# pxl-th/SLAM.jl

Measured on AMD Instinct MI355X. Metric: frames/sec KITTI-05 stereo @1k kpts; local-BA ms/iter for 50-KF window, higher is better.
Workload: dtype f64

## Files before the change

slam.jl_amd/csrc/detect.hip:

```cpp
#include "kpset.hpp"
#include "geom_device.hpp"
#include <cmath>
#include <cstddef>

#define DET_THREADS 256
#define DET_MAXCAND 512
#define DET_MAXTAPS 41
#define DET_MAXR 64

struct DetectArgs {
    const double *img; int H, W, pitch;
    const double *cur; int n_cur;
    int radius, grid_rows, grid_cols, cs, k;
    double min_response;
    int ntaps;
    double taps[DET_MAXTAPS];
    int64_t *cell_out;
    int *cell_cnt;
    const int *cur_off, *k_s; size_t zs; int kmax;
    const int *cur_cnt; int cur_stride, max_points;
    signed char lim[DET_MAXR + 1];
};
static void det_disk_table(DetectArgs &A)
{
    const int r = A.radius;
    for (int dy = 0; dy <= DET_MAXR; dy++) A.lim[dy] = -1;
    for (int dy = 0; dy <= r && dy <= DET_MAXR; dy++) {
        const volatile double a = (double)dy / (double)r;
        int lim = -1;
        for (int dx = 0; dx <= r; dx++) {
            const volatile double b = (double)dx / (double)r;
            const volatile double aa = a * a, bb = b * b;
            if (aa + bb < 1) lim = dx; else break;
        }
        A.lim[dy] = (signed char)lim;
    }
}

__device__ __forceinline__ int clampi(int v, int lo, int hi) { return v < lo ? lo : (v > hi ? hi : v); }

__device__ __forceinline__ double sep3(const double *src, int h, int w, int y, int x,
                                       double ky0, double ky1, double ky2, double kx0, double kx1, double kx2)
{
    const int ym = clampi(y - 1, 0, h - 1), yp = clampi(y + 1, 0, h - 1);
    double t[3];
#pragma unroll
    for (int j = 0; j < 3; j++) {
        const int xx = clampi(x + j - 1, 0, w - 1);
        double acc = 0.0;
        acc += src[ym + xx * h] * ky0; acc += src[y + xx * h] * ky1; acc += src[yp + xx * h] * ky2;
        t[j] = acc;
    }
    double acc = 0.0;
    acc += t[0] * kx0; acc += t[1] * kx1; acc += t[2] * kx2;
    return acc;
}

#define DET_SL 5
struct DetDiv {
    unsigned m, d;
    __device__ __forceinline__ explicit DetDiv(int dd) : m(0xffffffffu / (unsigned)(dd > 0 ? dd : 1) + 1u), d((unsigned)(dd > 0 ? dd : 1)) {}
    __device__ __forceinline__ int div(int i) const { return d == 1 ? i : (int)__umulhi((unsigned)i, m); }
    __device__ __forceinline__ int mod(int i) const { return i - div(i) * (int)d; }
};
template <int NT>
__device__ __forceinline__ void blur_mask(double *bA, double *T, const unsigned char *m0, const double *taps, int h, int w, int mh, int mw, int tid, const DetDiv &dns, const DetDiv &dh, int ntaps = NT)
{
    const int nt = NT > 0 ? NT : ntaps;
    if (NT > 0) {
        constexpr int NK = NT > 0 ? NT : 1;
        double k[NK];
#pragma unroll
        for (int j = 0; j < NK; j++) k[j] = taps[j];
        const int ns = (h + DET_SL - 1) / DET_SL;
        for (int it = tid; it < mw * ns; it += DET_THREADS) {
            const int tx = dns.div(it), ys = (it - tx * ns) * DET_SL;
            double v[DET_SL + NK - 1];
#pragma unroll
            for (int i = 0; i < DET_SL + NK - 1; i++) { const int yy = ys + i < mh ? ys + i : mh - 1; v[i] = (double)m0[yy + tx * mh]; }
#pragma unroll
            for (int q = 0; q < DET_SL; q++) {
                if (ys + q < h) {
                    double acc = 0.0;
#pragma unroll
                    for (int j = 0; j < NK; j++) acc += v[q + j] * k[j];
                    T[(ys + q) + tx * h] = acc;
                }
            }
        }
        __syncthreads();
        const int nsx = (w + DET_SL - 1) / DET_SL;
        for (int it = tid; it < h * nsx; it += DET_THREADS) {
            const int sx = dh.div(it), y = it - sx * h, xs = sx * DET_SL;
            double v[DET_SL + NK - 1];
#pragma unroll
            for (int i = 0; i < DET_SL + NK - 1; i++) { const int xx = xs + i < mw ? xs + i : mw - 1; v[i] = T[y + xx * h]; }
#pragma unroll
            for (int q = 0; q < DET_SL; q++) {
                if (xs + q < w) {
                    double acc = 0.0;
#pragma unroll
                    for (int j = 0; j < NK; j++) acc += v[q + j] * k[j];
                    bA[y + (xs + q) * h] = bA[y + (xs + q) * h] * acc;
                }
            }
        }
        return;
    }
    for (int i = tid; i < h * mw; i += DET_THREADS) {
        const int tx = dh.div(i), y = i - tx * h;
        double acc = 0.0;
        for (int j = 0; j < nt; j++) acc += (double)m0[(y + j) + tx * mh] * taps[j];
        T[i] = acc;
    }
    __syncthreads();
    for (int i = tid; i < h * w; i += DET_THREADS) {
        const int x = dh.div(i), y = i - x * h;
        double acc = 0.0;
        for (int j = 0; j < nt; j++) acc += T[y + (x + j) * h] * taps[j];
        bA[i] = bA[i] * acc;
    }
}

struct DetStrip { double v[3][DET_SL + 2]; };
__device__ __forceinline__ void det_strip_load(DetStrip &S, const double *src, int h, int w, int ys, int x)
{
    const int xm = clampi(x - 1, 0, w - 1), xp = clampi(x + 1, 0, w - 1);
#pragma unroll
    for (int i = 0; i < DET_SL + 2; i++) {
        const int yy = clampi(ys - 1 + i, 0, h - 1);
        S.v[0][i] = src[yy + xm * h]; S.v[1][i] = src[yy + x * h]; S.v[2][i] = src[yy + xp * h];
    }
}
__device__ __forceinline__ double det_strip_sep3(const DetStrip &S, int q, double ky0, double ky1, double ky2, double kx0, double kx1, double kx2)
{
    double t[3];
#pragma unroll
    for (int j = 0; j < 3; j++) {
        double acc = 0.0;
        acc += S.v[j][q] * ky0; acc += S.v[j][q + 1] * ky1; acc += S.v[j][q + 2] * ky2;
        t[j] = acc;
    }
    double acc = 0.0;
    acc += t[0] * kx0; acc += t[1] * kx1; acc += t[2] * kx2;
    return acc;
}

#ifdef DET_TRACE
#define DT(k) do { __syncthreads(); dt_clk[k] = clock64() - dt_t0; } while (0)
#else
#define DT(k)
#endif
#define SEL_NAME(k) k
#define SEL_ARG
#define SEL_STREAM(b) b
#include "detect_kernels.inc"
#undef SEL_NAME
#undef SEL_ARG
#undef SEL_STREAM
#define SEL_NAME(k) k##_sel
#define SEL_ARG , const int *stream_sel
#define SEL_STREAM(b) stream_sel[b]
#include "detect_kernels.inc"
#undef SEL_NAME
#undef SEL_ARG
#undef SEL_STREAM

__global__ __launch_bounds__(1024) void detect_compact(const int64_t *cell_out, const int *cell_cnt, int n_cells, int k,
                                                        int64_t *out , int cap,
                                                        const int *k_s )
{
    if (k_s) {
        const int z = blockIdx.x;
        cell_out += (size_t)z * n_cells * k * 2; cell_cnt += (size_t)z * n_cells; out += (size_t)z * (1 + 2 * (size_t)cap);
        k = k_s[z];
    }
    __shared__ int s_w[16];
    __shared__ int s_base;
    const int tid = threadIdx.x;
    if (tid == 0) s_base = 0;
    __syncthreads();
    for (int c0 = 0; c0 < n_cells; c0 += 1024) {
        const int c = c0 + tid, cnt = c < n_cells ? cell_cnt[c] : 0;
        const int start = cell_scan(cnt, s_w, &s_base);
        for (int i = 0; i < cnt; i++)
            if (start + i < cap) {
                out[1 + 2 * (start + i)] = cell_out[((size_t)c * k + i) * 2];
                out[2 + 2 * (start + i)] = cell_out[((size_t)c * k + i) * 2 + 1];
            }
    }
    if (tid == 0) out[0] = s_base;
}

static int det_plan(slam_ctx *ctx, DetectArgs &A, const double *img, int H, int W, int pitch, size_t zs, int max_points, int radius,
                    int grid_rows, int grid_cols, int cell_size, int kmax, double sigma_mask, double min_response, size_t *lds_bytes)
{
    A.img = img; A.H = H; A.W = W; A.pitch = pitch; A.zs = zs; A.radius = radius; det_disk_table(A);
    A.grid_rows = grid_rows; A.grid_cols = grid_cols; A.cs = cell_size; A.k = 0; A.kmax = kmax; A.n_cur = 0; A.min_response = min_response;
    A.cur = nullptr; A.cur_off = nullptr; A.k_s = nullptr; A.cur_cnt = nullptr; A.cur_stride = 0; A.max_points = max_points;
    A.ntaps = 0;
    if (sigma_mask != 0) {
        ARG_TRY(ctx, 4 * (int)std::ceil(sigma_mask) + 1 <= DET_MAXTAPS);
        A.ntaps = slam_gaussian_taps(sigma_mask, A.taps);
    }
    const int hw = A.ntaps >> 1;
    const size_t n = (size_t)cell_size * cell_size;
    const size_t mbytes = ((size_t)(cell_size + 2 * hw) * (cell_size + 2 * hw) + 7) & ~(size_t)7;
    ARG_TRY(ctx, mbytes <= n * 8 && (size_t)cell_size * (cell_size + 2 * hw) * 8 + mbytes <= 3 * n * 8);
    ARG_TRY(ctx, (size_t)kmax * sizeof(int) <= n * 8);
    *lds_bytes = 4 * n * sizeof(double);
    ARG_TRY(ctx, *lds_bytes <= 150 * 1024);
    HIP_TRY(ctx, hipFuncSetAttribute((const void *)detect_cells, hipFuncAttributeMaxDynamicSharedMemorySize, 150 * 1024));
    return SLAM_OK;
}

int slam_detect_device(slam_ctx *ctx, const double *img_dev, int H, int W, int pitch, const double *cur_yx, int n_cur,
                       int max_points, int radius, int grid_rows, int grid_cols, int cell_size,
                       double sigma_mask, double min_response, int64_t *out_rc, int cap, int *n_out)
{
    ARG_TRY(ctx, H > 0 && W > 0 && grid_rows > 0 && grid_cols > 0 && cell_size >= 8 && radius > 0 && radius <= DET_MAXR && n_out != nullptr);
    ARG_TRY(ctx, n_cur >= 0 && (n_cur == 0 || cur_yx != nullptr));
    *n_out = 0;
    if (n_cur >= max_points) return SLAM_OK;
    const int n_cells = grid_rows * grid_cols;
    const int n_detect = max_points - n_cur;
    const int k = (n_detect + n_cells - 1) / n_cells;
    DetectArgs A;
    size_t lds_bytes;
    int rc = det_plan(ctx, A, img_dev, H, W, pitch, 0, max_points, radius, grid_rows, grid_cols, cell_size, k, n_cur > 0 ? sigma_mask : 0.0, min_response, &lds_bytes);
    if (rc) return rc;
    A.k = k; A.n_cur = n_cur;
    const size_t out_pairs = (size_t)n_cells * k, out_b = 8 + out_pairs * 16;
    Layout D;
    const auto o_cur = D.take<double>((size_t)n_cur * 2); const auto o_cnt = D.take<int>(n_cells); const auto o_cout = D.take<int64_t>(out_pairs * 2), o_out = D.take<int64_t>(out_b / 8);
    char *s;
    rc = slam_scratch(ctx, D.size(), (void **)&s);
    if (rc) return rc;
    double *d_cur = o_cur.at(s); int *d_cnt = o_cnt.at(s);
    int64_t *d_cout = o_cout.at(s), *d_out = o_out.at(s);
    if (n_cur > 0) HIP_TRY(ctx, hipMemcpyAsync(d_cur, cur_yx, o_cur.bytes(), hipMemcpyHostToDevice, ctx->stream));
    A.cur = d_cur; A.cell_out = d_cout; A.cell_cnt = d_cnt;
    { ProfScope span(ctx, "detect");
      hipLaunchKernelGGL(detect_cells, dim3(n_cells), dim3(DET_THREADS), lds_bytes, ctx->stream, A);
      hipLaunchKernelGGL(detect_compact, dim3(1), dim3(1024), 0, ctx->stream, d_cout, d_cnt, n_cells, k, d_out, (int)out_pairs, (const int *)nullptr); }
    HIP_TRY(ctx, hipGetLastError());
    int64_t *h_out;
    rc = slam_pinned(ctx, out_b, (void **)&h_out);
    if (rc) return rc;
    HIP_TRY(ctx, hipMemcpyAsync(h_out, d_out, out_b, hipMemcpyDeviceToHost, ctx->stream));
    HIP_TRY(ctx, slam_stream_wait(ctx->stream));
    int64_t cnt = h_out[0];
    if (cnt > cap) return slam_fail(ctx, SLAM_ERR_CAPACITY, "slam_detect: %lld keypoints but cap = %d", (long long)cnt, cap);
    memcpy(out_rc, h_out + 1, (size_t)cnt * 16);
    *n_out = (int)cnt;
    return SLAM_OK;
}

extern "C" int slam_detect(slam_ctx *ctx, const double *image, int H, int W, const double *cur_yx, int n_cur,
                           int max_points, int radius, int grid_rows, int grid_cols, int cell_size,
                           double sigma_mask, double min_response, int64_t *out_rc, int cap, int *n_out)
{
    ARG_TRY(ctx, ctx != nullptr);
    ARG_TRY(ctx, image != nullptr && H > 0 && W > 0);
    HIP_TRY(ctx, hipSetDevice(ctx->device));
    void *d_img;
    int rc = slam_scratch2(ctx, (size_t)H * W * 8, &d_img);
    if (rc) return rc;
    HIP_TRY(ctx, hipMemcpyAsync(d_img, image, (size_t)H * W * 8, hipMemcpyHostToDevice, ctx->stream));
    return slam_detect_device(ctx, (const double *)d_img, H, W, H, cur_yx, n_cur, max_points, radius, grid_rows, grid_cols,
                              cell_size, sigma_mask, min_response, out_rc, cap, n_out);
}

extern "C" int slam_detect_pyr(slam_ctx *ctx, const slam_pyr *pyr, const double *cur_yx, int n_cur,
                               int max_points, int radius, int grid_rows, int grid_cols, int cell_size,
                               double sigma_mask, double min_response, int64_t *out_rc, int cap, int *n_out)
{
    ARG_TRY(ctx, ctx != nullptr && pyr != nullptr);
    HIP_TRY(ctx, hipSetDevice(ctx->device));
    return slam_detect_device(ctx, pyr->plane(0, 0), pyr->H[0], pyr->W[0], pyr->P[0], cur_yx, n_cur, max_points, radius, grid_rows,
                              grid_cols, cell_size, sigma_mask, min_response, out_rc, cap, n_out);
}

extern "C" int slam_detect_batch(slam_ctx *ctx, const slam_pyr *pyr0, int S, const double *cur_yx, const int32_t *cur_off,
                                 int max_points, int radius, int grid_rows, int grid_cols, int cell_size,
                                 double sigma_mask, double min_response, int64_t *out_rc, int cap, int32_t *out_off)
{
    ARG_TRY(ctx, ctx != nullptr && pyr0 != nullptr && S >= 1 && S <= 128 && cur_off != nullptr && out_off != nullptr);
    ARG_TRY(ctx, pyr0->batch_index == 0 && pyr0->batch_size == S);
    ARG_TRY(ctx, grid_rows > 0 && grid_cols > 0 && cell_size >= 8 && radius > 0 && radius <= DET_MAXR && cap >= 0 && (cap == 0 || out_rc != nullptr));
    HIP_TRY(ctx, hipSetDevice(ctx->device));
    const int n_cells = grid_rows * grid_cols, n_tot = cur_off[S];
    ARG_TRY(ctx, cur_off[0] == 0 && n_tot >= 0 && (n_tot == 0 || cur_yx != nullptr));
    int ks[128], kmax = 0;
    for (int s = 0; s < S; s++) {
        const int nc = cur_off[s + 1] - cur_off[s];
        ARG_TRY(ctx, nc >= 0);
        ks[s] = nc >= max_points ? 0 : (max_points - nc + n_cells - 1) / n_cells;
        kmax = ks[s] > kmax ? ks[s] : kmax;
    }
    for (int s = 0; s <= S; s++) out_off[s] = 0;
    if (kmax == 0) return SLAM_OK;
    DetectArgs A;
    size_t lds_bytes;
    int rc = det_plan(ctx, A, pyr0->plane(0, 0), pyr0->H[0], pyr0->W[0], pyr0->P[0], pyr0->zstride, max_points, radius, grid_rows, grid_cols, cell_size, kmax,
                      sigma_mask, min_response, &lds_bytes);
    if (rc) return rc;
    const size_t pairs = (size_t)n_cells * kmax, out_b = (size_t)S * (8 + pairs * 16);
    Layout D;
    const auto o_hdr = D.take<int>(512); const auto o_cur = D.take<double>((size_t)n_tot * 2); const size_t in_b = D.size();
    const auto o_cnt = D.take<int>((size_t)S * n_cells); const auto o_cout = D.take<int64_t>((size_t)S * pairs * 2), o_out = D.take<int64_t>(out_b / 8);
    char *d, *h;
    rc = slam_scratch(ctx, D.size(), (void **)&d);
    if (rc) return rc;
    rc = slam_pinned(ctx, in_b + out_b, (void **)&h);
    if (rc) return rc;
    memcpy(o_hdr.at(h), cur_off, (size_t)(S + 1) * 4); memcpy(o_hdr.at(h) + 256, ks, (size_t)S * 4);
    if (n_tot > 0) memcpy(o_cur.at(h), cur_yx, o_cur.bytes());
    HIP_TRY(ctx, hipMemcpyAsync(d, h, o_cur.off + o_cur.bytes(), hipMemcpyHostToDevice, ctx->stream));
    A.cur_off = o_hdr.at(d); A.k_s = o_hdr.at(d) + 256; A.cur = o_cur.at(d);
    A.cell_cnt = o_cnt.at(d); A.cell_out = o_cout.at(d);
    int64_t *d_out = o_out.at(d);
    { ProfScope span(ctx, "detect");
      hipLaunchKernelGGL(detect_cells, dim3(n_cells, S), dim3(DET_THREADS), lds_bytes, ctx->stream, A);
      hipLaunchKernelGGL(detect_compact, dim3(S), dim3(1024), 0, ctx->stream, (const int64_t *)A.cell_out, (const int *)A.cell_cnt, n_cells, kmax,
                         d_out, (int)pairs, A.k_s); }
    HIP_TRY(ctx, hipGetLastError());
    int64_t *h_out = (int64_t *)(h + in_b);
    HIP_TRY(ctx, hipMemcpyAsync(h_out, d_out, out_b, hipMemcpyDeviceToHost, ctx->stream));
    HIP_TRY(ctx, slam_stream_wait(ctx->stream));
    size_t tot = 0;
    for (int s = 0; s < S; s++) tot += (size_t)h_out[(size_t)s * (1 + 2 * pairs)];
    if (tot > (size_t)cap) return slam_fail(ctx, SLAM_ERR_CAPACITY, "slam_detect_batch: %zu keypoints but cap = %d", tot, cap);
    size_t o = 0;
    for (int s = 0; s < S; s++) {
        const int64_t *hs = h_out + (size_t)s * (1 + 2 * pairs);
        memcpy(out_rc + 2 * o, hs + 1, (size_t)hs[0] * 16);
        o += (size_t)hs[0]; out_off[s + 1] = (int32_t)o;
    }
    return SLAM_OK;
}

__global__ __launch_bounds__(64) void k_unselected_info(const uint8_t *mask, int S, const int *count, const int64_t *next_id, int *cnt0, int64_t *info)
{
    const int z = blockIdx.x * 64 + threadIdx.x;
    if (z >= S || mask[z]) return;
    cnt0[z] = count[z]; info[2 * z] = next_id[z]; info[2 * z + 1] = 0;
}

struct KpDetect { int max_points, radius, grid_rows, grid_cols, cell_size, n_cells, kmax; DetectArgs A; size_t lds_bytes; char *extra; };
static int kpset_detect_check(slam_ctx *ctx, const slam_kpset *ks, const slam_pyr *pyr0, int max_points, int radius, int grid_rows, int grid_cols, int cell_size, KpDetect &D)
{
    ARG_TRY(ctx, pyr0->batch_index == 0 && pyr0->batch_size >= ks->S);
    ARG_TRY(ctx, grid_rows > 0 && grid_cols > 0 && cell_size >= 8 && radius > 0 && radius <= DET_MAXR && max_points > 0);
    HIP_TRY(ctx, hipSetDevice(ctx->device));
    const int n_cells = grid_rows * grid_cols;
    ARG_TRY(ctx, ks->v.cap >= max_points + n_cells);
    D.max_points = max_points; D.radius = radius; D.grid_rows = grid_rows; D.grid_cols = grid_cols; D.cell_size = cell_size;
    D.n_cells = n_cells; D.kmax = (max_points + n_cells - 1) / n_cells;
    return SLAM_OK;
}
static int kpset_detect_plan(slam_ctx *ctx, const slam_kpset *ks, const slam_pyr *pyr0, double sigma_mask, double min_response, size_t extra, KpDetect &D)
{
    int rc = det_plan(ctx, D.A, pyr0->plane(0, 0), pyr0->H[0], pyr0->W[0], pyr0->P[0], pyr0->zstride, D.max_points, D.radius, D.grid_rows, D.grid_cols, D.cell_size,
                      D.kmax, sigma_mask, min_response, &D.lds_bytes);
    if (rc) return rc;
    D.A.cur = ks->v.yx; D.A.cur_cnt = ks->v.count; D.A.cur_stride = ks->v.cap;
    Layout L;
    const auto o_cnt = L.take<int>((size_t)ks->S * D.n_cells); const auto o_cout = L.take<int64_t>((size_t)ks->S * D.n_cells * D.kmax * 2); const auto o_extra = L.take<char>(extra);
    char *d;
    rc = slam_scratch(ctx, L.size(), (void **)&d);
    if (rc) return rc;
    D.A.cell_cnt = o_cnt.at(d); D.A.cell_out = o_cout.at(d); D.extra = o_extra.at(d);
    return SLAM_OK;
}
static void kpset_detect_append(slam_ctx *ctx, slam_kpset *ks, const KpDetect &D)
{
    if (const int *sel = kpset_sel_table(ks))
        hipLaunchKernelGGL(detect_append_sel, dim3(ks->n_sel), dim3(1024), 0, ctx->stream, (const int64_t *)D.A.cell_out, (const int *)D.A.cell_cnt, D.n_cells, D.kmax,
                           D.max_points, ks->v, ks->next_id, sel);
    else
        hipLaunchKernelGGL(detect_append, dim3(ks->S), dim3(1024), 0, ctx->stream, (const int64_t *)D.A.cell_out, (const int *)D.A.cell_cnt, D.n_cells, D.kmax,
                           D.max_points, ks->v, ks->next_id);
}
static int kpset_detect_cells(slam_ctx *ctx, const slam_kpset *ks, const KpDetect &D)
{
    if (const int *sel = kpset_sel_table(ks)) {
        HIP_TRY(ctx, hipFuncSetAttribute((const void *)detect_cells_sel, hipFuncAttributeMaxDynamicSharedMemorySize, 150 * 1024));
        hipLaunchKernelGGL(detect_cells_sel, dim3(D.n_cells, ks->n_sel), dim3(DET_THREADS), D.lds_bytes, ctx->stream, D.A, sel);
    } else
        hipLaunchKernelGGL(detect_cells, dim3(D.n_cells, ks->S), dim3(DET_THREADS), D.lds_bytes, ctx->stream, D.A);
    return SLAM_OK;
}

extern "C" int slam_kpset_detect(slam_ctx *ctx, slam_kpset *ks, const slam_pyr *pyr0, int max_points, int radius, int grid_rows, int grid_cols,
                                 int cell_size, double sigma_mask, double min_response)
{
    ARG_TRY(ctx, ctx != nullptr && ks != nullptr && pyr0 != nullptr);
    KpDetect D;
    int rc = kpset_detect_check(ctx, ks, pyr0, max_points, radius, grid_rows, grid_cols, cell_size, D);
    if (rc || kpset_none_selected(ks)) return rc;
    rc = kpset_detect_plan(ctx, ks, pyr0, sigma_mask, min_response, 0, D);
    if (rc) return rc;
    { ProfScope span(ctx, "detect");
      rc = kpset_detect_cells(ctx, ks, D);
      if (rc) return rc;
      kpset_detect_append(ctx, ks, D); }
    HIP_TRY(ctx, hipGetLastError());
    return SLAM_OK;
}

extern "C" int slam_kpset_detect_describe(slam_ctx *ctx, slam_kpset *ks, const slam_pyr *pyr0, int max_points, int radius, int grid_rows, int grid_cols,
                                          int cell_size, double sigma_mask, double min_response, const int32_t *pattern, int n_bits, double sigma,
                                          int window, uint64_t *desc_dev, int64_t *info_dev, int dcap)
{
    ARG_TRY(ctx, ctx != nullptr && ks != nullptr && pyr0 != nullptr && desc_dev != nullptr && info_dev != nullptr);
    const int S = ks->S;
    KpDetect D;
    int rc = kpset_detect_check(ctx, ks, pyr0, max_points, radius, grid_rows, grid_cols, cell_size, D);
    if (rc) return rc;
    if (dcap < D.n_cells * D.kmax)
        return slam_fail(ctx, SLAM_ERR_ARG, "slam_kpset_detect_describe: dcap = %d, a key-frame may append %d keypoints per stream", dcap, D.n_cells * D.kmax);
    BriefJob J;
    rc = brief_prepare(ctx, "slam_kpset_detect_describe", pyr0->plane(0, 0), pyr0->H[0], pyr0->W[0], pyr0->P[0], pyr0->zstride, pattern, n_bits,
                       sigma, window, &J);
    if (!rc) rc = kpset_detect_plan(ctx, ks, pyr0, sigma_mask, min_response, (size_t)S * 4, D);
    if (rc) return rc;
    int *cnt0 = (int *)D.extra;
    const int *sel = kpset_sel_table(ks);
    if (sel) {
        hipLaunchKernelGGL(k_unselected_info, dim3((S + 63) / 64), dim3(64), 0, ctx->stream, (const uint8_t *)ks->sel_mask, S, (const int *)ks->v.count,
                           (const int64_t *)ks->next_id, cnt0, info_dev);
        HIP_TRY(ctx, hipGetLastError());
        if (kpset_none_selected(ks)) return SLAM_OK;
    }
    { ProfScope span(ctx, "detect");
      { ProfScope cells(ctx, "detect_cells");
        rc = kpset_detect_cells(ctx, ks, D);
        if (rc) return rc; }
      if (sel)
          hipLaunchKernelGGL(detect_box_filter_sel, dim3((D.n_cells + 255) / 256, ks->n_sel), dim3(256), 0, ctx->stream, D.A.cell_out, D.A.cell_cnt, D.n_cells, D.kmax, max_points,
                             (const int *)ks->v.count, (const int64_t *)ks->next_id, pyr0->H[0], pyr0->W[0], (window + 1) / 2, cnt0, info_dev, sel);
      else
          hipLaunchKernelGGL(detect_box_filter, dim3((D.n_cells + 255) / 256, S), dim3(256), 0, ctx->stream, D.A.cell_out, D.A.cell_cnt, D.n_cells, D.kmax, max_points,
                             (const int *)ks->v.count, (const int64_t *)ks->next_id, pyr0->H[0], pyr0->W[0], (window + 1) / 2, cnt0, info_dev);
      kpset_detect_append(ctx, ks, D); }
    HIP_TRY(ctx, hipGetLastError());
    J.yx = ks->v.yx; J.cnt0 = cnt0; J.count = ks->v.count; J.cap = ks->v.cap; J.dcap = dcap; J.info = info_dev; J.out = desc_dev;
    return brief_launch(ctx, J, D.n_cells * D.kmax, S);
}
```

slam.jl_amd/csrc/detect_kernels.inc:

```

__global__ __launch_bounds__(DET_THREADS) void SEL_NAME(detect_cells)(DetectArgs A SEL_ARG)
{
    extern __shared__ double lds[];
#ifdef DET_TRACE
    long long dt_clk[12]; const long long dt_t0 = clock64();
    for (int q = 0; q < 12; q++) dt_clk[q] = 0;
#endif
    const double *a_img = A.img, *a_cur = A.cur;
    int a_ncur = A.n_cur, a_k = A.k;
    int64_t *a_cell_out = A.cell_out; int *a_cell_cnt = A.cell_cnt;
    if (A.cur_cnt) {
        const int z = SEL_STREAM(blockIdx.y), nc = A.grid_rows * A.grid_cols, ncur = A.cur_cnt[z];
        a_img += (size_t)z * A.zs; a_cur += 2 * (size_t)z * A.cur_stride; a_ncur = ncur;
        a_k = ncur >= A.max_points ? 0 : (A.max_points - ncur + nc - 1) / nc;
        a_cell_out += (size_t)z * nc * A.kmax * 2; a_cell_cnt += (size_t)z * nc;
    } else if (A.cur_off) {
        const int z = blockIdx.y, o = A.cur_off[z], nc = A.grid_rows * A.grid_cols;
        a_img += (size_t)z * A.zs; a_cur += 2 * (size_t)o; a_ncur = A.cur_off[z + 1] - o; a_k = A.k_s[z];
        a_cell_out += (size_t)z * nc * A.kmax * 2; a_cell_cnt += (size_t)z * nc;
    }
    const int cs = A.cs, H = A.H, W = A.W;
    const int cell = blockIdx.x;
    const int cyi = cell / A.grid_cols, cxi = cell % A.grid_cols;
    const int y0 = cyi * cs, x0 = cxi * cs;
    const int h = min(H, (cyi + 1) * cs) - y0, w = min(W, (cxi + 1) * cs) - x0;
    const int tid = threadIdx.x;
    const int n = cs * cs;
    double *bA = lds, *bB = lds + n, *bC = lds + 2 * n, *bD = lds + 3 * n;
    __shared__ int s_ncand, s_cnt;
    __shared__ __attribute__((aligned(16))) int s_cand[2 * DET_MAXCAND];
    __shared__ int s_lim[DET_MAXR + 1];
    __shared__ double s_taps[DET_MAXTAPS];

    if (h <= 0 || w <= 0 || a_k <= 0) { if (tid == 0) a_cell_cnt[cell] = 0; return; }

    if (a_ncur > 0 && A.ntaps > 0 && tid < A.ntaps) {
        const double *kt = (const double *)((const char *)__builtin_amdgcn_kernarg_segment_ptr() + offsetof(DetectArgs, taps));
        s_taps[tid] = kt[tid];
    }
    const DetDiv dvh(h), dnstr((h + DET_SL - 1) / DET_SL);
    for (int i0 = tid; i0 < h * w; i0 += 5 * DET_THREADS) {
        double v[5];
#pragma unroll
        for (int u = 0; u < 5; u++) {
            const int i = i0 + u * DET_THREADS, ic = i < h * w ? i : i0;
            const int icx = dvh.div(ic);
            v[u] = a_img[(size_t)(y0 + ic - icx * h) + (size_t)(x0 + icx) * A.pitch];
        }
#pragma unroll
        for (int u = 0; u < 5; u++) { const int i = i0 + u * DET_THREADS; if (i < h * w) bA[i] = v[u]; }
    }

    DT(0);
    if (a_ncur > 0) {
        const int hw = A.ntaps >> 1;
        const int mh = h + 2 * hw, mw = w + 2 * hw;
        const int r = A.radius;
        if (tid == 0) s_ncand = 0;
        if (tid <= r) s_lim[tid] = ((const signed char *)__builtin_amdgcn_kernarg_segment_ptr())[offsetof(DetectArgs, lim) + tid];
        __syncthreads();
        const int ylo = clampi(y0 - hw, 0, H - 1) + 1, yhi = clampi(y0 + h - 1 + hw, 0, H - 1) + 1;
        const int xlo = clampi(x0 - hw, 0, W - 1) + 1, xhi = clampi(x0 + w - 1 + hw, 0, W - 1) + 1;
        for (int k0 = tid; k0 < a_ncur; k0 += 4 * DET_THREADS) {
            double2 v[4];
#pragma unroll
            for (int u = 0; u < 4; u++) { const int k = k0 + u * DET_THREADS; v[u] = ((const double2 *)a_cur)[k < a_ncur ? k : k0]; }
#pragma unroll
            for (int u = 0; u < 4; u++) {
                const bool live = k0 + u * DET_THREADS < a_ncur;
                const long py = (long)rint(v[u].x), px = (long)rint(v[u].y);
                const bool hit = live && py + r >= ylo && py - r <= yhi && px + r >= xlo && px - r <= xhi;
                const unsigned long long bal = __ballot(hit);
                if (bal) {
                    int base = 0;
                    if ((tid & 63) == 0) base = atomicAdd(&s_ncand, __popcll(bal));
                    base = __shfl(base, 0);
                    const int slot = base + __popcll(bal & ((1ull << (tid & 63)) - 1ull));
                    if (hit && slot < DET_MAXCAND) { s_cand[2 * slot] = (int)py; s_cand[2 * slot + 1] = (int)px; }
                }
            }
        }
        __syncthreads();
        DT(1);
        const int ncand = s_ncand;
        const bool overflow = ncand > DET_MAXCAND;
        unsigned char *m0 = (unsigned char *)(lds + 4 * n) - ((mh * mw + 7) & ~7);
        if (!overflow) {
            for (int i = tid; i < mh * mw; i += DET_THREADS) m0[i] = 1;
            __syncthreads();
            const int nrow = 2 * r + 1, ty0 = y0 - hw, tx0 = x0 - hw;
            const DetDiv dnrow(nrow), dmh(mh);
            for (int q = tid; q < ncand * nrow; q += DET_THREADS) {
                const int c = dnrow.div(q), dyi = q - c * nrow - r;
                const int yy = s_cand[2 * c] + dyi, px = s_cand[2 * c + 1];
                const int lim = s_lim[abs(dyi)];
                const int ty = (yy - 1) - ty0;
                if (yy < 1 || yy > H || lim < 0 || ty < 0 || ty >= mh) continue;
                int txa = (max(px - lim, 1) - 1) - tx0, txb = (min(px + lim, W) - 1) - tx0;
                txa = txa < 0 ? 0 : txa; txb = txb > mw - 1 ? mw - 1 : txb;
                for (int tx = txa; tx <= txb; tx++) m0[ty + tx * mh] = 0;
            }
            __syncthreads();
            if (ty0 < 0 || ty0 + mh - 1 > H - 1 || tx0 < 0 || tx0 + mw - 1 > W - 1) {
                for (int i = tid; i < mh * mw; i += DET_THREADS) {
                    const int imx = dmh.div(i);
                    const int uy = ty0 + i - imx * mh, ux = tx0 + imx;
                    if (uy < 0 || uy > H - 1 || ux < 0 || ux > W - 1)
                        m0[i] = m0[(clampi(uy, 0, H - 1) - ty0) + (clampi(ux, 0, W - 1) - tx0) * mh];
                }
            }
        } else {
            for (int i = tid; i < mh * mw; i += DET_THREADS) {
                const int yy = clampi(y0 + i % mh - hw, 0, H - 1) + 1, xx = clampi(x0 + i / mh - hw, 0, W - 1) + 1;
                unsigned char m = 1;
                for (int c = 0; c < a_ncur; c++) {
                    long py = (long)rint(a_cur[2 * c]), px = (long)rint(a_cur[2 * c + 1]);
                    const long dy = labs(yy - py), dx = labs(xx - px);
                    if (dy <= r && dx <= s_lim[dy]) { m = 0; break; }
                }
                m0[i] = m;
            }
        }
        DT(2);
        __syncthreads();
        if (A.ntaps > 0) {
            double *T = bB;
            if (A.ntaps == 13) blur_mask<13>(bA, T, m0, s_taps, h, w, mh, mw, tid, dnstr, dvh);
            else blur_mask<0>(bA, T, m0, s_taps, h, w, mh, mw, tid, dnstr, dvh, A.ntaps);
        } else {
            for (int i = tid; i < h * w; i += DET_THREADS) {
                const int x = dvh.div(i), y = i - x * h;
                bA[i] = bA[i] * (double)m0[(y + hw) + (x + hw) * mh];
            }
        }
    }
    __syncthreads();

    DT(3);
    const int nstr = (h + DET_SL - 1) / DET_SL;
    for (int it = tid; it < w * nstr; it += DET_THREADS) {
        const int x = dnstr.div(it), ys = (it - x * nstr) * DET_SL;
        DetStrip S;
        det_strip_load(S, bA, h, w, ys, x);
#pragma unroll
        for (int q = 0; q < DET_SL; q++) {
            if (ys + q < h) {
                const double g1 = det_strip_sep3(S, q, -1.0 / 2, 0.0 / 2, 1.0 / 2, 1.0 / 4, 2.0 / 4, 1.0 / 4);
                const double g2 = det_strip_sep3(S, q, 1.0 / 4, 2.0 / 4, 1.0 / 4, -1.0 / 2, 0.0 / 2, 1.0 / 2);
                const int i = (ys + q) + x * h;
                bB[i] = g1 * g1; bC[i] = g1 * g2; bD[i] = g2 * g2;
            }
        }
    }
    __syncthreads();
    DT(4);
    double *resp = bA;
    for (int it = tid; it < w * nstr; it += DET_THREADS) {
        const int x = dnstr.div(it), ys = (it - x * nstr) * DET_SL;
        double xx[DET_SL], xy[DET_SL], yy[DET_SL];
        DetStrip S;
        det_strip_load(S, bB, h, w, ys, x);
#pragma unroll
        for (int q = 0; q < DET_SL; q++) xx[q] = det_strip_sep3(S, q, 1.0 / 3, 1.0 / 3, 1.0 / 3, 1.0 / 3, 1.0 / 3, 1.0 / 3);
        det_strip_load(S, bC, h, w, ys, x);
#pragma unroll
        for (int q = 0; q < DET_SL; q++) xy[q] = det_strip_sep3(S, q, 1.0 / 3, 1.0 / 3, 1.0 / 3, 1.0 / 3, 1.0 / 3, 1.0 / 3);
        det_strip_load(S, bD, h, w, ys, x);
#pragma unroll
        for (int q = 0; q < DET_SL; q++) yy[q] = det_strip_sep3(S, q, 1.0 / 3, 1.0 / 3, 1.0 / 3, 1.0 / 3, 1.0 / 3, 1.0 / 3);
#pragma unroll
        for (int q = 0; q < DET_SL; q++) {
            if (ys + q < h) {
                const double dd = xx[q] - yy[q];
                resp[(ys + q) + x * h] = ((xx[q] + yy[q]) - sqrt(dd * dd + 4 * (xy[q] * xy[q]))) / 2;
            }
        }
    }
    __syncthreads();
    DT(5);

    int *mx_idx = (int *)bC;
    double *mx_val = bD;
    if (tid == 0) { s_cnt = 0; s_ncand = 0; }
    __syncthreads();
    for (int it0 = 0; it0 < w * nstr; it0 += DET_THREADS) {
        const int it = it0 + tid;
        const bool act = it < w * nstr;
        const int x = act ? dnstr.div(it) : 0, ys = act ? (it - x * nstr) * DET_SL : 0;
        DetStrip S;
        det_strip_load(S, resp, h, w, ys, x);
        const bool cl = x > 0, cr = x < w - 1;
#pragma unroll
        for (int q = 0; q < DET_SL; q++) {
            const int y = ys + q;
            const double c = S.v[1][q + 1];
            bool ismax = act && y < h;
            const bool ru = y > 0, rd = y < h - 1;
            if (cl) { if (ru && !(S.v[0][q] < c)) ismax = false; if (!(S.v[0][q + 1] < c)) ismax = false; if (rd && !(S.v[0][q + 2] < c)) ismax = false; }
            if (ru && !(S.v[1][q] < c)) ismax = false;
            if (rd && !(S.v[1][q + 2] < c)) ismax = false;
            if (cr) { if (ru && !(S.v[2][q] < c)) ismax = false; if (!(S.v[2][q + 1] < c)) ismax = false; if (rd && !(S.v[2][q + 2] < c)) ismax = false; }
            const unsigned long long bal = __ballot(ismax);
            if (bal) {
                int base = 0;
                if ((tid & 63) == 0) base = atomicAdd(&s_ncand, __popcll(bal));
                base = __shfl(base, 0);
                const int slot = base + __popcll(bal & ((1ull << (tid & 63)) - 1ull));
                if (ismax) { mx_idx[slot] = y + x * h; mx_val[slot] = c; }
            }
        }
    }
    __syncthreads();

    DT(6);
    int *sel = (int *)bB;
    if (tid < 64) {
        const int nmx = s_ncand;
        int cnt = 0;
        for (int round = 0; round < a_k; round++) {
            double bv = -INFINITY; int bi = 0x7fffffff, bs = -1;
            for (int j = tid; j < nmx; j += 64) {
                const int i = mx_idx[j];
                if (i >= 0) {
                    const double v = mx_val[j];
                    if (v > bv || (v == bv && i < bi)) { bv = v; bi = i; bs = j; }
                }
            }
            for (int off = 32; off >= 1; off >>= 1) {
                const double ov = __shfl_xor(bv, off); const int oi = __shfl_xor(bi, off), os = __shfl_xor(bs, off);
                if (oi != 0x7fffffff && (bi == 0x7fffffff || ov > bv || (ov == bv && oi < bi))) { bv = ov; bi = oi; bs = os; }
            }
            if (bi == 0x7fffffff) break;
            if (tid == 0) {
                mx_idx[bs] = -1;
                if (!(bv < A.min_response)) sel[cnt] = bi;
            }
            if (!(bv < A.min_response)) cnt++;
        }
        if (tid == 0) s_cnt = cnt;
    }
    __syncthreads();

    DT(7);
    if (tid == 0) {
        int cnt = s_cnt;
        for (int i = 1; i < cnt; i++) { int v = sel[i], j = i - 1; while (j >= 0 && sel[j] > v) { sel[j + 1] = sel[j]; j--; } sel[j + 1] = v; }
        int64_t *o = a_cell_out + (size_t)cell * a_k * 2;
        for (int i = 0; i < cnt; i++) {
            int y = sel[i] % h, x = sel[i] / h;
            o[2 * i] = y + 1 + y0; o[2 * i + 1] = x + 1 + x0;
        }
        a_cell_cnt[cell] = cnt;
    }
#ifdef DET_TRACE
    DT(8);
    if (tid == 0 && cell == 200 && blockIdx.y == 3) printf("detect cell: ncur %d k %d | tile %lld scan %lld raster %lld blur %lld grad %lld resp %lld lmax %lld topk %lld emit %lld cycles\n", a_ncur, a_k, dt_clk[0], dt_clk[1] - dt_clk[0], dt_clk[2] - dt_clk[1], dt_clk[3] - dt_clk[2], dt_clk[4] - dt_clk[3], dt_clk[5] - dt_clk[4], dt_clk[6] - dt_clk[5], dt_clk[7] - dt_clk[6], dt_clk[8] - dt_clk[7]);
#endif
}

__global__ __launch_bounds__(1024) void SEL_NAME(detect_append)(const int64_t *cell_out, const int *cell_cnt, int n_cells, int kmax, int max_points, KpsetView K,
                                                                int64_t *next_id SEL_ARG)
{
    const int z = SEL_STREAM(blockIdx.x), cap = K.cap;
    cell_out += (size_t)z * n_cells * kmax * 2; cell_cnt += (size_t)z * n_cells;
    const size_t b = (size_t)z * cap;
    const int n0 = K.count[z];
    const int64_t id0 = next_id[z];
    __shared__ int s_w[16];
    __shared__ int s_base;
    const int tid = threadIdx.x;
    if (tid == 0) s_base = 0;
    __syncthreads();
    if (n0 >= max_points) return;
    const int kz = (max_points - n0 + n_cells - 1) / n_cells;
    for (int c0 = 0; c0 < n_cells; c0 += 1024) {
        const int c = c0 + tid, cnt = c < n_cells ? cell_cnt[c] : 0;
        const int start = cell_scan(cnt, s_w, &s_base);
        for (int i = 0; i < cnt; i++) {
            const int j = n0 + start + i;
            if (j < cap) {
                const size_t q = b + j;
                K.yx[2 * q] = (double)cell_out[((size_t)c * kz + i) * 2]; K.yx[2 * q + 1] = (double)cell_out[((size_t)c * kz + i) * 2 + 1];
                K.syx[2 * q] = 0.0; K.syx[2 * q + 1] = 0.0; K.xyz[3 * q] = 0.0; K.xyz[3 * q + 1] = 0.0; K.xyz[3 * q + 2] = 0.0;
                K.id[q] = id0 + start + i; K.is3d[q] = 0; K.stereo[q] = 0; K.haskf[q] = 0;
            }
        }
    }
    if (tid == 0) { const int n1 = n0 + s_base; K.count[z] = n1 < cap ? n1 : cap; next_id[z] = id0 + s_base; }
}

__global__ __launch_bounds__(256) void SEL_NAME(detect_box_filter)(int64_t *cell_out, int *cell_cnt, int n_cells, int kmax, int max_points, const int *count,
                                                                   const int64_t *next_id, int H, int W, int lim, int *cnt0, int64_t *info SEL_ARG)
{
    const int z = SEL_STREAM(blockIdx.y), c = blockIdx.x * 256 + threadIdx.x;
    const int n0 = count[z];
    if (c == 0) { cnt0[z] = n0; info[2 * z] = next_id[z]; }
    if (c >= n_cells || n0 >= max_points) return;
    const int kz = (max_points - n0 + n_cells - 1) / n_cells;
    int64_t *o = cell_out + ((size_t)z * n_cells * kmax + (size_t)c * kz) * 2;
    int *pc = cell_cnt + (size_t)z * n_cells + c;
    const int cnt = *pc;
    int m = 0;
    for (int i = 0; i < cnt; i++) {
        const int64_t y = o[2 * i], x = o[2 * i + 1];
        if (y - lim < 1 || y + lim > H || x - lim < 1 || x + lim > W) continue;
        o[2 * m] = y; o[2 * m + 1] = x; m++;
    }
    *pc = m;
}
```

Measured before the change: 24700.

## Shrink detector LDS footprint and pin occupancy to five waves per EU

Reworks the per-cell Shi-Tomasi pipeline so it needs three LDS planes instead of four when every strip item fits in a single pass over the threads. In that case the last product plane and the response stay in registers and are written back after a barrier. The candidate buffer is aliased into a plane, and the Sobel and box-filter passes are restructured as column-wise accumulation with scheduling fences. The kernel is also constrained to 5 waves per EU. The aim is more resident blocks through lower LDS and register use. The risks are extra barriers, aliasing hazards between reused buffers, and register spills forced by the wave cap.

Measured after the change: 24720 (median of 3 runs). No clear change (+0.1%).

```diff
diff --git a/slam.jl_amd/csrc/detect.hip b/slam.jl_amd/csrc/detect.hip
--- a/slam.jl_amd/csrc/detect.hip
+++ b/slam.jl_amd/csrc/detect.hip
@@ -63,6 +63,14 @@
     __device__ __forceinline__ int div(int i) const { return d == 1 ? i : (int)__umulhi((unsigned)i, m); }
     __device__ __forceinline__ int mod(int i) const { return i - div(i) * (int)d; }
 };
+__host__ __device__ __forceinline__ int det_mask_off(int cs, int hw) { const int t = cs * (cs + 2 * hw); return t > DET_MAXCAND ? t : DET_MAXCAND; }
+__host__ __device__ __forceinline__ bool det_four_planes(int cs) { return cs * ((cs + DET_SL - 1) / DET_SL) > DET_THREADS; }
+static size_t det_lds_bytes(int cs, int hw)
+{
+    const size_t n = (size_t)cs * cs, mbytes = ((size_t)(cs + 2 * hw) * (cs + 2 * hw) + 7) & ~(size_t)7;
+    const size_t region = (size_t)det_mask_off(cs, hw) * 8 + mbytes, planes = (det_four_planes(cs) ? 3 : 2) * n * 8;
+    return n * 8 + (region > planes ? region : planes);
+}
 template <int NT>
 __device__ __forceinline__ void blur_mask(double *bA, double *T, const unsigned char *m0, const double *taps, int h, int w, int mh, int mw, int tid, const DetDiv &dns, const DetDiv &dh, int ntaps = NT)
 {
@@ -132,19 +140,35 @@
         S.v[0][i] = src[yy + xm * h]; S.v[1][i] = src[yy + x * h]; S.v[2][i] = src[yy + xp * h];
     }
 }
-__device__ __forceinline__ double det_strip_sep3(const DetStrip &S, int q, double ky0, double ky1, double ky2, double kx0, double kx1, double kx2)
-{
-    double t[3];
-#pragma unroll
-    for (int j = 0; j < 3; j++) {
-        double acc = 0.0;
-        acc += S.v[j][q] * ky0; acc += S.v[j][q + 1] * ky1; acc += S.v[j][q + 2] * ky2;
-        t[j] = acc;
-    }
-    double acc = 0.0;
-    acc += t[0] * kx0; acc += t[1] * kx1; acc += t[2] * kx2;
-    return acc;
-}
+__device__ __forceinline__ void det_strip_zero(double *acc)
+{
+#pragma unroll
+    for (int q = 0; q < DET_SL; q++) acc[q] = 0.0;
+}
+__device__ __forceinline__ void det_col_load(double *v, const double *col, int h, int ys)
+{
+#pragma unroll
+    for (int i = 0; i < DET_SL + 2; i++) v[i] = col[clampi(ys - 1 + i, 0, h - 1)];
+}
+__device__ __forceinline__ void det_col_acc(double *acc, const double *v, double ky0, double ky1, double ky2, double kx)
+{
+#pragma unroll
+    for (int q = 0; q < DET_SL; q++) {
+        double t = 0.0;
+        t += v[q] * ky0; t += v[q + 1] * ky1; t += v[q + 2] * ky2;
+        acc[q] += t * kx;
+    }
+}
+__device__ __forceinline__ void det_strip_store(double *dst, const double *keep, int h, int items, int tid, const DetDiv &dns)
+{
+    if (tid >= items) return;
+    const int x = dns.div(tid), ys = (tid - x * (int)dns.d) * DET_SL;
+#pragma unroll
+    for (int q = 0; q < DET_SL; q++)
+        if (ys + q < h) dst[(ys + q) + x * h] = keep[q];
+}
+#define DET_WAVES 5
+#define DET_FENCE() __builtin_amdgcn_sched_barrier(0)
 
 #ifdef DET_TRACE
 #define DT(k) do { __syncthreads(); dt_clk[k] = clock64() - dt_t0; } while (0)
@@ -205,10 +229,9 @@
     }
     const int hw = A.ntaps >> 1;
     const size_t n = (size_t)cell_size * cell_size;
-    const size_t mbytes = ((size_t)(cell_size + 2 * hw) * (cell_size + 2 * hw) + 7) & ~(size_t)7;
-    ARG_TRY(ctx, mbytes <= n * 8 && (size_t)cell_size * (cell_size + 2 * hw) * 8 + mbytes <= 3 * n * 8);
-    ARG_TRY(ctx, (size_t)kmax * sizeof(int) <= n * 8);
-    *lds_bytes = 4 * n * sizeof(double);
+    const size_t nmx = (size_t)((cell_size + 1) / 2) * ((cell_size + 1) / 2);
+    ARG_TRY(ctx, (size_t)kmax * sizeof(int) <= n * 8 && nmx * (sizeof(double) + sizeof(int)) <= n * 8);
+    *lds_bytes = det_lds_bytes(cell_size, hw);
     ARG_TRY(ctx, *lds_bytes <= 150 * 1024);
     HIP_TRY(ctx, hipFuncSetAttribute((const void *)detect_cells, hipFuncAttributeMaxDynamicSharedMemorySize, 150 * 1024));
     return SLAM_OK;
diff --git a/slam.jl_amd/csrc/detect_kernels.inc b/slam.jl_amd/csrc/detect_kernels.inc
--- a/slam.jl_amd/csrc/detect_kernels.inc
+++ b/slam.jl_amd/csrc/detect_kernels.inc
@@ -1,5 +1,5 @@
 
-__global__ __launch_bounds__(DET_THREADS) void SEL_NAME(detect_cells)(DetectArgs A SEL_ARG)
+__global__ __launch_bounds__(DET_THREADS) __attribute__((amdgpu_waves_per_eu(DET_WAVES, DET_WAVES))) void SEL_NAME(detect_cells)(DetectArgs A SEL_ARG)
 {
     extern __shared__ double lds[];
 #ifdef DET_TRACE
@@ -26,9 +26,10 @@
     const int h = min(H, (cyi + 1) * cs) - y0, w = min(W, (cxi + 1) * cs) - x0;
     const int tid = threadIdx.x;
     const int n = cs * cs;
-    double *bA = lds, *bB = lds + n, *bC = lds + 2 * n, *bD = lds + 3 * n;
+    double *bA = lds, *b1 = lds + n, *b2 = lds + 2 * n;
+    const bool four = det_four_planes(cs);
     __shared__ int s_ncand, s_cnt;
-    __shared__ __attribute__((aligned(16))) int s_cand[2 * DET_MAXCAND];
+    int *s_cand = (int *)b1;
     __shared__ int s_lim[DET_MAXR + 1];
     __shared__ double s_taps[DET_MAXTAPS];
 
@@ -84,7 +85,7 @@
         DT(1);
         const int ncand = s_ncand;
         const bool overflow = ncand > DET_MAXCAND;
-        unsigned char *m0 = (unsigned char *)(lds + 4 * n) - ((mh * mw + 7) & ~7);
+        unsigned char *m0 = (unsigned char *)(b1 + det_mask_off(cs, hw));
         if (!overflow) {
             for (int i = tid; i < mh * mw; i += DET_THREADS) m0[i] = 1;
             __syncthreads();
@@ -124,7 +125,7 @@
         DT(2);
         __syncthreads();
         if (A.ntaps > 0) {
-            double *T = bB;
+            double *T = b1;
             if (A.ntaps == 13) blur_mask<13>(bA, T, m0, s_taps, h, w, mh, mw, tid, dnstr, dvh);
             else blur_mask<0>(bA, T, m0, s_taps, h, w, mh, mw, tid, dnstr, dvh, A.ntaps);
         } else {
@@ -138,49 +139,70 @@
 
     DT(3);
     const int nstr = (h + DET_SL - 1) / DET_SL;
+    double *p22 = four ? lds + 3 * n : bA;
+    double keep[DET_SL];
+#pragma unroll
+    for (int q = 0; q < DET_SL; q++) keep[q] = 0.0;
     for (int it = tid; it < w * nstr; it += DET_THREADS) {
         const int x = dnstr.div(it), ys = (it - x * nstr) * DET_SL;
-        DetStrip S;
-        det_strip_load(S, bA, h, w, ys, x);
+        double g1[DET_SL], g2[DET_SL];
+        det_strip_zero(g1); det_strip_zero(g2);
+#pragma unroll
+        for (int j = 0; j < 3; j++) {
+            double v[DET_SL + 2];
+            det_col_load(v, bA + clampi(x + j - 1, 0, w - 1) * h, h, ys);
+            det_col_acc(g1, v, -1.0 / 2, 0.0 / 2, 1.0 / 2, j == 1 ? 2.0 / 4 : 1.0 / 4);
+            det_col_acc(g2, v, 1.0 / 4, 2.0 / 4, 1.0 / 4, j == 0 ? -1.0 / 2 : (j == 1 ? 0.0 / 2 : 1.0 / 2));
+            DET_FENCE();
+        }
 #pragma unroll
         for (int q = 0; q < DET_SL; q++) {
             if (ys + q < h) {
-                const double g1 = det_strip_sep3(S, q, -1.0 / 2, 0.0 / 2, 1.0 / 2, 1.0 / 4, 2.0 / 4, 1.0 / 4);
-                const double g2 = det_strip_sep3(S, q, 1.0 / 4, 2.0 / 4, 1.0 / 4, -1.0 / 2, 0.0 / 2, 1.0 / 2);
                 const int i = (ys + q) + x * h;
-                bB[i] = g1 * g1; bC[i] = g1 * g2; bD[i] = g2 * g2;
-            }
-        }
+                b1[i] = g1[q] * g1[q]; b2[i] = g1[q] * g2[q]; keep[q] = g2[q] * g2[q];
+                if (four) p22[i] = keep[q];
+            }
+        }
+    }
+    if (!four) {
+        __syncthreads();
+        det_strip_store(p22, keep, h, w * nstr, tid, dnstr);
     }
     __syncthreads();
     DT(4);
-    double *resp = bA;
+    double *resp = four ? bA : b1;
     for (int it = tid; it < w * nstr; it += DET_THREADS) {
         const int x = dnstr.div(it), ys = (it - x * nstr) * DET_SL;
         double xx[DET_SL], xy[DET_SL], yy[DET_SL];
-        DetStrip S;
-        det_strip_load(S, bB, h, w, ys, x);
-#pragma unroll
-        for (int q = 0; q < DET_SL; q++) xx[q] = det_strip_sep3(S, q, 1.0 / 3, 1.0 / 3, 1.0 / 3, 1.0 / 3, 1.0 / 3, 1.0 / 3);
-        det_strip_load(S, bC, h, w, ys, x);
-#pragma unroll
-        for (int q = 0; q < DET_SL; q++) xy[q] = det_strip_sep3(S, q, 1.0 / 3, 1.0 / 3, 1.0 / 3, 1.0 / 3, 1.0 / 3, 1.0 / 3);
-        det_strip_load(S, bD, h, w, ys, x);
-#pragma unroll
-        for (int q = 0; q < DET_SL; q++) yy[q] = det_strip_sep3(S, q, 1.0 / 3, 1.0 / 3, 1.0 / 3, 1.0 / 3, 1.0 / 3, 1.0 / 3);
+        det_strip_zero(xx); det_strip_zero(xy); det_strip_zero(yy);
+#pragma unroll 1
+        for (int j = 0; j < 3; j++) {
+            const int xc = clampi(x + j - 1, 0, w - 1) * h;
+            double v[DET_SL + 2];
+            det_col_load(v, b1 + xc, h, ys); det_col_acc(xx, v, 1.0 / 3, 1.0 / 3, 1.0 / 3, 1.0 / 3); DET_FENCE();
+            det_col_load(v, b2 + xc, h, ys); det_col_acc(xy, v, 1.0 / 3, 1.0 / 3, 1.0 / 3, 1.0 / 3); DET_FENCE();
+            det_col_load(v, p22 + xc, h, ys); det_col_acc(yy, v, 1.0 / 3, 1.0 / 3, 1.0 / 3, 1.0 / 3); DET_FENCE();
+        }
 #pragma unroll
         for (int q = 0; q < DET_SL; q++) {
             if (ys + q < h) {
                 const double dd = xx[q] - yy[q];
-                resp[(ys + q) + x * h] = ((xx[q] + yy[q]) - sqrt(dd * dd + 4 * (xy[q] * xy[q]))) / 2;
-            }
-        }
+                keep[q] = ((xx[q] + yy[q]) - sqrt(dd * dd + 4 * (xy[q] * xy[q]))) / 2;
+                if (four) resp[(ys + q) + x * h] = keep[q];
+            }
+            DET_FENCE();
+        }
+    }
+    if (!four) {
+        __syncthreads();
+        det_strip_store(resp, keep, h, w * nstr, tid, dnstr);
     }
     __syncthreads();
     DT(5);
 
-    int *mx_idx = (int *)bC;
-    double *mx_val = bD;
+    const int nmx_cap = ((cs + 1) >> 1) * ((cs + 1) >> 1);
+    double *mx_val = b2;
+    int *mx_idx = (int *)(b2 + nmx_cap);
     if (tid == 0) { s_cnt = 0; s_ncand = 0; }
     __syncthreads();
     for (int it0 = 0; it0 < w * nstr; it0 += DET_THREADS) {
@@ -213,7 +235,7 @@
     __syncthreads();
 
     DT(6);
-    int *sel = (int *)bB;
+    int *sel = (int *)(four ? b1 : bA);
     if (tid < 64) {
         const int nmx = s_ncand;
         int cnt = 0;
```
